# EnriqueOO97/MultiModalVC

Measured on NVIDIA B200. Metric: AV-HuBERT-L encoder 6s-clips/sec, higher is better.
Workload: dtype bf16

## Files before the change

### include/avh_b200.h

```cpp
#ifndef AVH_B200_H_
#define AVH_B200_H_

#include <stdint.h>

#ifdef __cplusplus
extern "C" {
#endif

#define AVH_ABI_VERSION 1
#if defined(__GNUC__)
#define AVH_API __attribute__((visibility("default")))
#else
#define AVH_API
#endif

enum { AVH_F32 = 0, AVH_F16 = 1, AVH_BF16 = 2, AVH_U8 = 3  };
enum {
  AVH_COMPUTE_BF16 = 0,
  AVH_COMPUTE_FP32 = 1
};
enum { AVH_FUSE_CONCAT = 0, AVH_FUSE_ADD = 1 };

typedef struct avh_config {
  int32_t encoder_layers;
// ... 81 lines not shown
                                const int32_t* len_queries, int B, int Lq, int Lk, void* out, int out_dtype, void* stream);

AVH_API int avh_forward_ragged(avh_handle* h, const void* video, int video_dtype, const void* audio, int audio_dtype,
                               const int64_t* audio_strides, const int32_t* lengths, int B, int T, int output_layer,
                               void* out, int out_dtype, void* stream);

AVH_API int avh_set_video_preprocess(avh_handle* h, int src_h, int src_w, double mean, double std);

AVH_API int avh_video_preprocess(const uint8_t* frames, int64_t n_frames, int src_h, int src_w, int crop, double mean,
                         double std, void* out, int out_dtype, void* stream);

AVH_API int avh_forward_host(avh_handle* h, const void* video, int video_dtype, const void* audio, int audio_dtype,
                     const uint8_t* padding_mask, int B, int T, int output_layer, void* out, int out_dtype,
                     void* stream);

AVH_API int avh_forward_host_async(avh_handle* h, const void* video, int video_dtype, const void* audio, int audio_dtype,
                           const uint8_t* padding_mask, int B, int T, int output_layer, void* out, int out_dtype,
                           void* stream);

AVH_API int avh_read_stage(avh_handle* h, const char* name, float* dst, int64_t capacity_elems, void* stream);

AVH_API int avh_fbank(const int16_t* wav, const int64_t* offsets, const int32_t* video_len, int n_clips, int T,
              int normalize, float* out, uint8_t* padding_mask, void* stream);

AVH_API int avh_add_noise(const int16_t* wav, const int64_t* offsets, int n_clips, const float* noise, int64_t noise_len,
                  float snr_db, int16_t* out, double* scratch, void* stream);

AVH_API int avh_attention_bf16(const void* qkv, const uint8_t* padding_mask, const int32_t* cu_rows, int64_t rows, int B,
                               int T, int D, int H, int impl, void* out, void* stream);

AVH_API int avh_gemm_bf16(const void* A, const void* B, int64_t M, int N, int K, const float* bias, int gelu,
                  const void* R, int r_fp32, void* C, int c_fp32, int block_n, int pair, int occ, void* stream);

AVH_API int avh_gemm_set_trace(void* dev_buf);

AVH_API int avh_set_profiling(avh_handle* h, int on);
AVH_API int avh_profile_json(avh_handle* h, char* buf, int64_t cap);

AVH_API int64_t avh_launch_count(void);
AVH_API void avh_reset_launch_count(void);
AVH_API int64_t avh_graph_launch_count(void);

#ifdef __cplusplus
}
#endif
#endif
```

### multimodalvc_b200/_lib.py

```python
import ctypes
import os

_HERE = os.path.dirname(os.path.abspath(__file__))
LIB_PATH = os.path.join(_HERE, "libavh_b200.so")

AVH_F32, AVH_F16, AVH_BF16, AVH_U8 = 0, 1, 2, 3
AVH_COMPUTE_BF16, AVH_COMPUTE_FP32 = 0, 1
AVH_FUSE_CONCAT, AVH_FUSE_ADD = 0, 1

EXPORTS = [
    "avh_abi_version", "avh_last_error", "avh_create", "avh_destroy", "avh_load_tensor", "avh_finalize_weights",
    "avh_forward", "avh_forward_host", "avh_forward_host_async", "avh_read_stage", "avh_fbank", "avh_add_noise", "avh_gemm_bf16",
    "avh_launch_count", "avh_reset_launch_count", "avh_set_profiling", "avh_profile_json",
    "avh_gemm_set_trace", "avh_set_video_preprocess", "avh_video_preprocess", "avh_drop_host_weights",
    "avh_release_stream", "avh_attention_bf16", "avh_forward_ragged", "avh_encoder_forward", "avh_forward_train", "avh_bn_stats_count", "avh_read_bn_stats", "avh_dropout", "avh_interp_linear", "avh_graph_launch_count",
    "avh_mask_substitute", "avh_compute_logits", "avh_sum_squares", "avh_qformer_forward",
    "avh_encoder_grad_count", "avh_encoder_train_forward", "avh_encoder_backward",
    "avh_encoder_backward_buckets", "avh_grad_bucket_count", "avh_grad_bucket_range", "avh_grad_bucket_wait",
    "avh_refresh_weights_device",
    "avh_tail_grad_count", "avh_tail_train_forward", "avh_full_grad_count", "avh_full_train_forward",
]


class AvhConfig(ctypes.Structure):
    _fields_ = [
        ("encoder_layers", ctypes.c_int32),
        ("encoder_embed_dim", ctypes.c_int32),
        ("encoder_ffn_embed_dim", ctypes.c_int32),
        ("encoder_attention_heads", ctypes.c_int32),
        ("audio_feat_dim", ctypes.c_int32),
        ("modality_fuse", ctypes.c_int32),
        ("layer_norm_first", ctypes.c_int32),
        ("conv_pos", ctypes.c_int32),
        ("conv_pos_groups", ctypes.c_int32),
        ("compute_mode", ctypes.c_int32),
        ("frontend_chunk_frames", ctypes.c_int32),
        ("capture_stages", ctypes.c_int32),
        ("reserved", ctypes.c_int32 * 4),
    ]


class AvhTrainArgs(ctypes.Structure):
    _fields_ = [
        ("dropout_input", ctypes.c_float),
        ("dropout", ctypes.c_float),
# ... 30 lines not shown
    lib.avh_forward_ragged.argtypes = [vp, vp, i32, vp, i32, ctypes.POINTER(i64), ctypes.POINTER(ctypes.c_int32), i32, i32, i32, vp,
                                       i32, vp]
    lib.avh_forward_train.argtypes = [vp, vp, i32, vp, i32, ctypes.POINTER(i64), vp, i32, i32, i32, ctypes.POINTER(AvhTrainArgs),
                                      vp, i32, vp]
    lib.avh_interp_linear.argtypes = [vp, i32, i32, i32, i32, vp, vp, i32, vp, vp, vp]
    lib.avh_encoder_grad_count.argtypes = [vp, ctypes.POINTER(i64)]
    lib.avh_tail_grad_count.argtypes = [vp, ctypes.POINTER(i64)]
    lib.avh_full_grad_count.argtypes = [vp, i32, i32, ctypes.POINTER(i64)]
    lib.avh_full_train_forward.argtypes = [vp, vp, i32, vp, i32, ctypes.POINTER(i64), vp, i32, i32, ctypes.c_float, ctypes.c_float,
                                           vp, i32, vp]
    lib.avh_tail_train_forward.argtypes = [vp, vp, i32, vp, i32, i32, vp, i32, vp]
    lib.avh_encoder_train_forward.argtypes = [vp, vp, i32, vp, i32, i32, vp, i32, vp]
    lib.avh_encoder_backward.argtypes = [vp, vp, i32, vp, i32, vp, i64, vp]
    lib.avh_encoder_backward_buckets.argtypes = [vp, vp, i32, vp, i32, vp, i32, i64, vp]
    lib.avh_grad_bucket_count.argtypes = [vp, ctypes.POINTER(ctypes.c_int32)]
    lib.avh_grad_bucket_range.argtypes = [vp, i32, ctypes.POINTER(i64), ctypes.POINTER(i64)]
    lib.avh_grad_bucket_wait.argtypes = [vp, i32, vp]
    lib.avh_refresh_weights_device.argtypes = [vp, ctypes.POINTER(ctypes.c_char_p), ctypes.POINTER(vp), ctypes.POINTER(ctypes.c_int32),
                                               ctypes.POINTER(i64), i32, vp]
    lib.avh_qformer_forward.argtypes = [vp, vp, i32, vp, ctypes.POINTER(ctypes.c_int32), i32, i32, i32, vp, i32, vp]
    lib.avh_mask_substitute.argtypes = [vp, i32, i32, ctypes.POINTER(i64), i32, i32, i32, vp, vp, i32, vp, vp, i32, vp]
    lib.avh_compute_logits.argtypes = [vp, i32, i64, vp, i32, i64, vp, i64, i32, i32, i32, ctypes.c_float, vp, i64, vp]
    lib.avh_sum_squares.argtypes = [vp, i32, i64, vp, vp]
    lib.avh_dropout.argtypes = [vp, i32, i64, ctypes.c_float, ctypes.c_uint64, ctypes.c_uint32, vp]
    lib.avh_bn_stats_count.argtypes = [vp, ctypes.POINTER(i64)]
    lib.avh_read_bn_stats.argtypes = [vp, vp, i64, vp]
    lib.avh_encoder_forward.argtypes = [vp, vp, i32, vp, i32, i32, i32, vp, i32, vp]
    lib.avh_forward_host.argtypes = [vp, vp, i32, vp, i32, vp, i32, i32, i32, vp, i32, vp]
    lib.avh_forward_host_async.argtypes = [vp, vp, i32, vp, i32, vp, i32, i32, i32, vp, i32, vp]
    lib.avh_read_stage.argtypes = [vp, ctypes.c_char_p, vp, i64, vp]
    lib.avh_fbank.argtypes = [vp, vp, vp, i32, i32, i32, vp, vp, vp]
    lib.avh_add_noise.argtypes = [vp, vp, i32, vp, i64, ctypes.c_float, vp, vp, vp]
    lib.avh_gemm_bf16.argtypes = [vp, vp, i64, i32, i32, vp, i32, vp, i32, vp, i32, i32, i32, i32, vp]
    lib.avh_attention_bf16.argtypes = [vp, vp, vp, i64, i32, i32, i32, i32, i32, vp, vp]
    lib.avh_gemm_set_trace.argtypes = [vp]
    lib.avh_set_video_preprocess.argtypes = [vp, i32, i32, ctypes.c_double, ctypes.c_double]
    lib.avh_video_preprocess.argtypes = [vp, i64, i32, i32, i32, ctypes.c_double, ctypes.c_double, vp, i32, vp]
    lib.avh_set_profiling.argtypes = [vp, i32]
    lib.avh_profile_json.argtypes = [vp, ctypes.c_char_p, i64]
    lib.avh_launch_count.restype = i64
    lib.avh_reset_launch_count.restype = None
    lib.avh_graph_launch_count.restype = i64
    for name in EXPORTS:
        fn = getattr(lib, name)
        if fn.restype is ctypes.c_int and name not in ("avh_abi_version",):
            fn.restype = i32
    if lib.avh_abi_version() != 1:
        raise RuntimeError("libavh_b200.so ABI version mismatch; rebuild with `python -m multimodalvc_b200.build --force`")
    _lib = lib
    return lib


def check(status):
    if status != 0:
        msg = load().avh_last_error()
        raise RuntimeError("libavh_b200: " + (msg.decode() if msg else "unknown error"))


def launch_count():
    return int(load().avh_launch_count())


def reset_launch_count():
    load().avh_reset_launch_count()
```

### multimodalvc_b200/csrc/api.cu

```cuda
#include "avh_b200.h"
#include "common.cuh"
#include "gemm.h"
#include "kernels.h"

#include <array>
#include <atomic>
#include <cmath>
#include <cstdlib>
#include <cstring>
#include <functional>
#include <map>
#include <tuple>
#include <memory>
#include <mutex>
#include <string>
#include <vector>

#include <cuda_fp16.h>

namespace avh {

static thread_local std::string g_err;
void set_last_error(const std::string& msg) { g_err = msg; }
static std::atomic<long long> g_launches{0};
// ... 144 lines not shown
  bool has_video = false, has_audio = false, has_mask = false;
  bool train = false;
  float p_in = 0.f, p_enc = 0.f, p_act = 0.f, bn_momentum = 0.1f;
  unsigned long long seed = 0;
  std::vector<unsigned char> layer_skip;
  bool enc_only = false;
  bool enc_train = false;
  int tail = 0;
  size_t fwd_steps = 0;
  float* grads = nullptr;
  long long grad_floats = 0;
  float* dx_out = nullptr;
  float* dy_in = nullptr;
  float fgm = 1.f;
  bool fwd_done = false;
  int Lk = 0;
  unsigned char* qmask_dev = nullptr;
  unsigned char* kmask_dev = nullptr;
  bool ragged = false;
  long long Nb = 0;
  int* rag = nullptr;
  int rag_ints = 0, rag_items_off = 0, rag_max_items = 0;
  static constexpr int RAG_SLOTS = 4;
  int* rag_host[RAG_SLOTS] = {nullptr, nullptr, nullptr, nullptr};
  cudaEvent_t rag_done[RAG_SLOTS] = {nullptr, nullptr, nullptr, nullptr};
  struct GradBucket { long long begin, end; cudaEvent_t ev; };
  std::vector<GradBucket> buckets;
  int rag_next = 0;
  int* pos_row_map = nullptr;

  Arena arena;
  std::vector<Step> steps;
  std::vector<GemmPlan*> gemms;
  std::vector<ConvWinPlan*> convwins;
  std::vector<ConvFramePlan*> convframes;
  StemFusedPlan stemf;
  AttnTcPlan att;
  std::map<std::string, std::pair<const void*, std::pair<int, long long>>> stages;
  CallArgs args;
  struct Segment { size_t begin, end; cudaGraphExec_t exec; int kernels; };
  std::vector<Segment> segments;
  bool segments_ready = false;
  unsigned char* mask_dev = nullptr;
  int direct_runs = 0;
  long long last_use = 0;
  cudaStream_t stream = nullptr;
  void drop_graphs() {
    for (auto& sg : segments)
      if (sg.exec) cudaGraphExecDestroy(sg.exec);
    segments.clear();
    segments_ready = false;
  }
  ~Plan() {
    drop_graphs();
    for (GemmPlan* g : gemms) delete g;
    for (ConvWinPlan* g : convwins) delete g;
    for (ConvFramePlan* g : convframes) delete g;
    for (int i = 0; i < RAG_SLOTS; ++i) {
      if (rag_host[i]) cudaFreeHost(rag_host[i]);
      if (rag_done[i]) cudaEventDestroy(rag_done[i]);
    }
    for (GradBucket& gb : buckets)
      if (gb.ev) cudaEventDestroy(gb.ev);
    arena.release();
  }
};

}
}

using namespace avh;

struct avh_handle {
  avh_config cfg;
  int device = 0;
  int P = 1;
  bool finalized = false;
  std::map<std::string, HostTensor> raw;
  Arena warena;
  ConvUnit stem;
  PackedW stem_wf;
  BlockW blocks[4][2];
  LinearW proj_v, proj_a, post_proj;
  LinearW post_projT;
  LinearW proj_vT;
  bool has_post_proj = false;
  float *fuse_ln_g = nullptr, *fuse_ln_b = nullptr, *enc_ln_g = nullptr, *enc_ln_b = nullptr;
  PackedW pos_w;
// ... 1026 lines not shown
    void* ol = f32 ? nullptr : hbuf.data;
    b.tag = "layer_ln";
    b.push([=](cudaStream_t s) { return launch_layernorm(src, DT_F32, D, g, be, 1e-5f, of, ol, DT_BF16, nullptr, N, D, s); });
    if (f32 && also_f32 != nullptr) {
      float* hd = reinterpret_cast<float*>(hbuf.data);
      b.push([=](cudaStream_t s) {
        return cudaMemcpyAsync(also_f32, hd, (size_t)N * D * 4, cudaMemcpyDeviceToDevice, s) == cudaSuccess ? 0 : 1;
      });
    }
    sync_op(hbuf);
  };
  auto x_to_h = [&]() {
    void* dst = hbuf.op;
    const int planes = P;
    b.tag = "split";
    b.push([=](cudaStream_t s) { return launch_split_rows(x, D, dst, planes, N, D, 0, 0, s); });
  };

  if (!c.layer_norm_first) {
    float* g = h->enc_ln_g; float* be = h->enc_ln_b;
    b.tag = "layer_ln";
    b.push([=](cudaStream_t s) { return launch_layernorm(x, DT_F32, D, g, be, 1e-5f, x, nullptr, DT_BF16, nullptr, N, D, s); });
    if (!train) x_to_h();
  }
  if (train) {
    b.tag = "dropout";
    b.push([=](cudaStream_t s) {
      return pl->p_enc > 0.f ? launch_dropout(x, DT_F32, nullptr, N * D, pl->p_enc, pl->seed, 2u, s) : 0;
    });
    if (!c.layer_norm_first) x_to_h();
  }
  const int n_layers = plan->output_layer > 0 ? std::min(plan->output_layer, c.encoder_layers) : c.encoder_layers;
  const bool att_tc = !f32 && (rg || T > 96) && (size_t)((T + 127) / 128 * 128) * 4 <= 48 * 1024;
  for (int l = 0; l < n_layers; ++l) {
    const LayerW& lw = h->layers[l];
    b.cur_layer = l;
    if (c.layer_norm_first) ln_to_h(x, lw.ln1_g, lw.ln1_b, nullptr);
    {
      Epilogue ep = ep_base(qkv.data, 3 * D);
      ep.col_bias = lw.qkv.bias;
      b.tag = "qkv_proj";
      if (!b.gemm(hbuf.op, N, P * D, lw.qkv.w, N, {Tap{0, 0, 0}}, D / 64, D, ep)) return false;
    }
    {
      const void* q = qkv.data; void* o = ctx.data;
      b.tag = "attention";
      const double att_flops = 4.0 * (double)B * Hh * (double)T * (double)T * 64.0;
      if (att_tc) {
        if (!sizing && l == 0 && attention_tc_plan(q, N, B, T, D, Hh, &plan->att)) return false;
        b.push([=](cudaStream_t s) {
          return attention_tc_launch(pl->att, hm ? pl->mask_dev : nullptr, pl->ragged ? pl->rag + 16 : nullptr, o, s);
        }, att_flops);
      } else {
        b.push([=](cudaStream_t s) {
          return launch_attention(q, hm ? pl->mask_dev : nullptr, o, B, T, D, Hh, f32 ? 1 : 0, s);
        }, att_flops);
      }
      sync_op(ctx);
    }
    auto dropout_add = [&](unsigned site) {
      float* target = c.layer_norm_first ? x : tmp;
      b.tag = "dropout";
      if (!c.layer_norm_first)
        b.push([=](cudaStream_t s) {
          return cudaMemcpyAsync(tmp, x, (size_t)N * D * 4, cudaMemcpyDeviceToDevice, s) == cudaSuccess ? 0 : 1;
        });
      b.push([=](cudaStream_t s) { return launch_dropout(target, DT_F32, dtmp, N * D, pl->p_enc, pl->seed, site, s); });
    };
    {
      Epilogue ep;
      ep.C = c.layer_norm_first ? x : tmp; ep.ldc = D; ep.c_fp32 = 1;
      ep.col_bias = lw.out.bias; ep.R = x; ep.ldr = D; ep.r_fp32 = 1;
      if (train) { ep.C = dtmp; ep.R = nullptr; }
      b.tag = "out_proj";
      if (!b.gemm(ctx.op, N, P * D, lw.out.w, N, {Tap{0, 0, 0}}, D / 64, D, ep)) return false;
      if (train) dropout_add(16u + 4u * (unsigned)l);
    }
    if (c.layer_norm_first) ln_to_h(x, lw.ln2_g, lw.ln2_b, nullptr);
    else {
      float* g = lw.ln1_g; float* be = lw.ln1_b;
      b.tag = "layer_ln";
      b.push([=](cudaStream_t s) { return launch_layernorm(tmp, DT_F32, D, g, be, 1e-5f, x, nullptr, DT_BF16, nullptr, N, D, s); });
      x_to_h();
    }
    {
      Epilogue ep = ep_base(ffn.data, F);
      ep.col_bias = lw.fc1.bias; ep.act = ACT_GELU;
      b.tag = "fc1";
      if (!b.gemm(hbuf.op, N, P * D, lw.fc1.w, N, {Tap{0, 0, 0}}, D / 64, D, ep)) return false;
      if (train) {
        void* fd = ffn.data;
        const unsigned site = 17u + 4u * (unsigned)l;
        b.tag = "dropout";
        b.push([=](cudaStream_t s) {
          return pl->p_act > 0.f ? launch_dropout(fd, act_dt, nullptr, N * F, pl->p_act, pl->seed, site, s) : 0;
        });
      }
      sync_op(ffn);
    }
    {
      Epilogue ep;
      ep.C = c.layer_norm_first ? x : tmp; ep.ldc = D; ep.c_fp32 = 1;
      ep.col_bias = lw.fc2.bias; ep.R = x; ep.ldr = D; ep.r_fp32 = 1;
      if (train) { ep.C = dtmp; ep.R = nullptr; }
      b.tag = "fc2";
      if (!b.gemm(ffn.op, N, P * F, lw.fc2.w, N, {Tap{0, 0, 0}}, F / 64, F, ep)) return false;
      if (train) dropout_add(18u + 4u * (unsigned)l);
    }
    if (!c.layer_norm_first) {
      float* g = lw.ln2_g; float* be = lw.ln2_b;
      b.tag = "layer_ln";
      b.push([=](cudaStream_t s) { return launch_layernorm(tmp, DT_F32, D, g, be, 1e-5f, x, nullptr, DT_BF16, nullptr, N, D, s); });
      if (l + 1 < n_layers) x_to_h();
    }
  }
  b.cur_layer = -1;
  b.tag = "final_ln";
  if (rg) {
    float* y = x;
    if (c.layer_norm_first && plan->output_layer == 0) {
      y = reinterpret_cast<float*>(b.alloc((size_t)N * D * 4));
      float* g = h->enc_ln_g; float* be = h->enc_ln_b;
      b.push([=](cudaStream_t s) { return launch_layernorm(x, DT_F32, D, g, be, 1e-5f, y, nullptr, DT_BF16, nullptr, N, D, s); });
    }
    b.tag = "unpack";
    b.cur_direct = true;
    b.push([=](cudaStream_t s) {
      return launch_unpack_rows(y, pl->rag + 16, pl->args.out, pl->args.out_dt, B, pl->args.pitch, D, s);
    });
  } else
  if (c.layer_norm_first && plan->output_layer == 0) {
    b.cur_direct = true;
    float* g = h->enc_ln_g; float* be = h->enc_ln_b;
    b.push([=](cudaStream_t s) {
      return launch_layernorm(x, DT_F32, D, g, be, 1e-5f, nullptr, pl->args.out, pl->args.out_dt, nullptr, N, D, s);
    });
  } else {
    b.cur_direct = true;
    b.push([=](cudaStream_t s) { return launch_convert(x, DT_F32, pl->args.out, pl->args.out_dt, N * D, s); });
  }
// ... 2020 lines not shown
    std::vector<avh::KStep> t;
    for (int i = 0; i < kb0 * r; ++i) t.push_back(avh::KStep{(i % kb0) * 64, 0, (i % kb0) * 64, 0});
    if (d_ktab == nullptr) AVH_CUDA_OK(cudaMalloc(&d_ktab, avh::GEMM_MAX_KSTEPS * sizeof(avh::KStep)));
    AVH_CUDA_OK(cudaMemcpy(d_ktab, t.data(), t.size() * sizeof(avh::KStep), cudaMemcpyHostToDevice));
    pr.ktable = reinterpret_cast<const avh::KStep*>(d_ktab);
    pr.num_kb = kb0 * r;
  }
  pr.block_n = block_n;
  pr.pair = pair;
  pr.occ = occ;
  {
    static std::map<int, std::pair<float*, int*>> ws;
    int dev = 0;
    AVH_CUDA_OK(cudaGetDevice(&dev));
    const size_t bytes = (size_t)avh::device_sm_count() * 128 * 256 * 4;
    if (ws.find(dev) == ws.end()) {
      float* w = nullptr; int* f = nullptr;
      AVH_CUDA_OK(cudaMalloc(&w, bytes));
      AVH_CUDA_OK(cudaMalloc(&f, 4096));
      AVH_CUDA_OK(cudaMemset(f, 0, 4096));
      ws[dev] = {w, f};
    }
    pr.sk_ws = ws[dev].first; pr.sk_ws_bytes = bytes; pr.sk_flags = ws[dev].second;
  }
  pr.ep.C = C; pr.ep.ldc = N; pr.ep.c_fp32 = c_fp32;
  pr.ep.col_bias = bias;
  pr.ep.act = gelu ? avh::ACT_GELU : avh::ACT_NONE;
  pr.ep.R = R; pr.ep.ldr = N; pr.ep.r_fp32 = r_fp32;
  avh::GemmPlan plan;
  if (avh::gemm_plan(pr, &plan)) return 1;
  return avh::gemm_launch(plan, reinterpret_cast<cudaStream_t>(stream));
}

}
```

### multimodalvc_b200/csrc/gemm.h

```cpp
#pragma once
#include <cuda.h>
#include <cuda_runtime.h>
#include <vector_types.h>
#include <stdint.h>

#include <vector>

namespace avh {

enum { ACT_NONE = 0, ACT_GELU = 1, ACT_PRELU = 2 };
enum { MAP_IDENTITY = 0, MAP_2LEVEL = 1 };

struct Epilogue {
  void* C = nullptr;
  long long ldc = 0;
  int c_fp32 = 0;
  const float* col_scale = nullptr;
  const float* col_bias = nullptr;
  int act = ACT_NONE;
  const float* slope1 = nullptr;
  const void* R = nullptr;
  long long ldr = 0;
  int r_fp32 = 0;
  const float* slope2 = nullptr;
// ... 86 lines not shown
struct ConvFramePlan {
  CUtensorMap tma_a, tma_b, tma_c, tma_a2;
  ConvFrameProblem prob;
  int grid = 0, stages = 0, pair = 1;
  size_t smem = 0;
  std::vector<int> tiles_host;
  const int* tiles_dev = nullptr;
};
int conv_frame_plan(const ConvFrameProblem& prob, ConvFramePlan* plan);
size_t conv_frame_table_bytes(const ConvFrameProblem& prob);
int conv_frame_bind_table(ConvFramePlan* plan, void* dev_table);
int conv_frame_launch(const ConvFramePlan& plan, cudaStream_t stream);
struct StemFusedPlan {
  const void* w = nullptr;
};
int stem_fused_plan(const void* w_packed, StemFusedPlan* plan);
int stem_fused_launch(const StemFusedPlan& plan, const void* video, int in_dt, int T, int b0, int nb, const float* scale,
                      const float* bias, const float* slope, void* pooled_out, cudaStream_t stream);
struct AttnTcPlan {
  CUtensorMap tma_q, tma_kv;
  int B = 0, T = 0, D = 0, H = 0;
  int kv_rows = 0, stages = 0, stage_bytes = 0, mask_floats = 0;
  size_t smem = 0;
};
int attention_tc_plan(const void* qkv, long long rows, int B, int T, int D, int H, AttnTcPlan* plan);
int attention_tc_launch(const AttnTcPlan& plan, const unsigned char* kpm, const int* cu, void* out, cudaStream_t stream);
int stem_fused_ragged_items(const int* lengths, int n_clips, int sms, int4* items, int max_items);
int stem_fused_launch_ragged(const StemFusedPlan& plan, const void* video, int in_dt, int Tpitch, const int4* items,
                             const int* n_items, const int* cu, const float* scale, const float* bias, const float* slope,
                             void* out, cudaStream_t stream);
int encode_2d(CUtensorMap* map, const void* base, long long rows, int cols, long long ld, int box_rows);
int encode_c(CUtensorMap* map, const void* base, long long rows, int cols, long long ld, int fp32);

constexpr int GEMM_MAX_KSTEPS = 768;

int gemm_plan(const GemmProblem& prob, GemmPlan* plan);
int gemm_launch(const GemmPlan& plan, cudaStream_t stream);
int gemm_pick_block_n(long long M, int N);
void gemm_set_trace(unsigned long long* dev_buf);

}
```

### multimodalvc_b200/csrc/gemm_tcgen05.cu

```cuda
#include "common.cuh"
#include "gemm.h"

#include <cstdlib>
#include <mutex>
#include <set>

namespace avh {

namespace {

constexpr int BM = 128;
constexpr int BK = 64;
constexpr int A_STAGE_BYTES = BM * BK * 2;
constexpr int MAX_STAGES = 8;
constexpr int COLVEC_BYTES = 2 * 4 * 256 * 4;
constexpr int BAR_BYTES = (2 * MAX_STAGES + 4) * 8 + 16;

template <int OCC>
struct Occ {
  static constexpr int EPI_WARPS = OCC == 2 ? 4 : 8;
  static constexpr int NUM_THREADS = 128 + 32 * EPI_WARPS;
  static constexpr int TMEM_COLS = 512 / OCC;
  static constexpr int ACC_STRIDE = 256 / OCC;
  static constexpr int EPI_STAGE_BYTES = EPI_WARPS * 4096;
  static constexpr int SMEM_LIMIT = OCC == 2 ? 113 * 1024 : 227 * 1024;
  static constexpr int HSTRIDE = EPI_WARPS / 4;
};

struct KernelParams {
  long long M;
  int N;
  int num_kb;
  int num_m_blk, num_n_blk;
  int block_n;
  int stages;
  int ktab_bytes;
  int a_col_per_nblk;
  const int* a_col_nblk;
// ... 569 lines not shown
          __syncwarp();
        }
        if (half >= nchunks) {
          tc_fence_before();
          __syncwarp();
          if (lane == 0) {
            if (PAIR == 2) mbar_arrive_leader(&tmem_empty[acc]);
            else mbar_arrive(&tmem_empty[acc]);
          }
        }
      }
      if (warp == 4 && lane == 0) {
        if (it == 0) AVH_TRACE(7);
        AVH_TRACE(9);
      }
      if (SK != 0 && sk_last >= sk_first) {
        asm volatile("bar.sync 1, %0;" ::"n"(32 * EPI_WARPS) : "memory");
        if (threadIdx.x == 128)
          for (int v = sk_first; v <= sk_last; ++v) p.sk_flags[v * PAIR + cta_rank] = 0;
      }
    }
    if (lane == 0 && p.c_mode != 0) tma_wait_group0();
  }

  tc_fence_before();
  if (PAIR == 2) cluster_sync_all();
  else __syncthreads();
  tc_fence_after();
  if (threadIdx.x == 0) AVH_TRACE(10);
  if (warp == 2) {
    if (PAIR == 2) tmem_dealloc_pair(tmem_base, TMEM_COLS);
    else tmem_dealloc(tmem_base, TMEM_COLS);
    if (lane == 0) AVH_TRACE(11);
  }
}

typedef CUresult (*EncodeTiledFn)(CUtensorMap*, CUtensorMapDataType, cuuint32_t, void*, const cuuint64_t*,
                                  const cuuint64_t*, const cuuint32_t*, const cuuint32_t*, CUtensorMapInterleave,
                                  CUtensorMapSwizzle, CUtensorMapL2promotion, CUtensorMapFloatOOBfill);

EncodeTiledFn get_encode_fn() {
  static EncodeTiledFn fn = nullptr;
  if (fn == nullptr) {
    void* p = nullptr;
    cudaDriverEntryPointQueryResult q;
    if (cudaGetDriverEntryPoint("cuTensorMapEncodeTiled", &p, cudaEnableDefault, &q) == cudaSuccess &&
        q == cudaDriverEntryPointSuccess)
      fn = reinterpret_cast<EncodeTiledFn>(p);
  }
  return fn;
}

}

int encode_c(CUtensorMap* map, const void* base, long long rows, int cols, long long ld, int fp32) {
  EncodeTiledFn fn = get_encode_fn();
  AVH_CHECK(fn != nullptr, "cuTensorMapEncodeTiled entry point not available");
  const int es = fp32 ? 4 : 2;
  AVH_CHECK((reinterpret_cast<uintptr_t>(base) & 15) == 0 && (ld * es) % 16 == 0, "TMA store alignment");
  cuuint64_t dims[2] = {(cuuint64_t)cols, (cuuint64_t)rows};
  cuuint64_t strides[1] = {(cuuint64_t)ld * es};
  cuuint32_t box[2] = {(cuuint32_t)(128 / es), 32u};
  cuuint32_t estr[2] = {1, 1};
  CUresult r = fn(map, fp32 ? CU_TENSOR_MAP_DATA_TYPE_FLOAT32 : CU_TENSOR_MAP_DATA_TYPE_BFLOAT16, 2,
                  const_cast<void*>(base), dims, strides, box, estr, CU_TENSOR_MAP_INTERLEAVE_NONE,
                  CU_TENSOR_MAP_SWIZZLE_128B, CU_TENSOR_MAP_L2_PROMOTION_NONE, CU_TENSOR_MAP_FLOAT_OOB_FILL_NONE);
// ... 214 lines not shown
    fn = gemm_kernel<1, O, A, R, S, C, F>;
  AVH_SPEC(1, ACT_NONE, 0, 0, 0, 0)
  AVH_SPEC(1, ACT_NONE, 0, 0, 0, 1)
  AVH_SPEC(1, ACT_GELU, 0, 0, 0, 0)
  AVH_SPEC(1, ACT_GELU, 0, 0, 0, 1)
  AVH_SPEC(1, ACT_NONE, 1, 0, 0, 1)
  AVH_SPEC(1, ACT_GELU, 1, 0, 0, 1)
  AVH_SPEC(1, ACT_PRELU, 0, 0, 1, 0)
  AVH_SPEC(1, ACT_PRELU, 0, 0, 1, 1)
  AVH_SPEC(1, ACT_NONE, 1, 1, 1, 0)
  AVH_SPEC(1, ACT_NONE, 1, 1, 1, 1)
  AVH_SPEC(1, ACT_NONE, 0, 0, 1, 0)
  AVH_SPEC(1, ACT_NONE, 0, 0, 1, 1)
  AVH_SPEC(2, ACT_NONE, 0, 0, 0, 0)
  AVH_SPEC(2, ACT_NONE, 0, 0, 0, 1)
  AVH_SPEC(2, ACT_GELU, 0, 0, 0, 0)
  AVH_SPEC(2, ACT_NONE, 1, 0, 0, 1)
  AVH_SPEC(2, ACT_GELU, 1, 0, 0, 1)
  AVH_SPEC(2, ACT_PRELU, 0, 0, 1, 0)
  AVH_SPEC(2, ACT_NONE, 1, 1, 1, 0)
  AVH_SPEC(2, ACT_NONE, 0, 0, 1, 0)
#undef AVH_SPEC
  if (fn == nullptr) {
    if (pair == 2) fn = gemm_kernel<2, 1, -1, -1, -1, -1, -1>;
    else if (occ == 2) fn = gemm_kernel<1, 2, -1, -1, -1, -1, -1>;
    else fn = gemm_kernel<1, 1, -1, -1, -1, -1, -1>;
  }
  if (ensure_dyn_smem(reinterpret_cast<const void*>(fn), occ == 2 ? Occ<2>::SMEM_LIMIT : Occ<1>::SMEM_LIMIT)) return 1;
  AVH_CUDA_OK(cudaLaunchKernelEx(&cfg, fn, plan.tma_a, plan.tma_b, plan.tma_c, kp));
  count_launch(1);
  return 0;
}

}
```

Before: 4232.

## Fuse FFN fc1 and fc2 into one persistent kernel with row-level dependencies

Replaces the two separate fc1 (GELU) and fc2 (bias plus residual) GEMM launches in inference with a single persistent tcgen05 kernel. Tiles come from an atomic work queue and are interleaved with a planned lag, so fc2 tiles for an M row-block start once all of that block's fc1 tiles are published through per-row release/acquire counters. This removes the inter-kernel drain and tail between the two GEMMs and lets the two phases overlap. The cost is spin-waiting, a global atomic scheduler, a self-resetting sync buffer, and a heuristic tile-size and lag model.

```diff
diff --git a/include/avh_b200.h b/include/avh_b200.h
--- a/include/avh_b200.h
+++ b/include/avh_b200.h
@@ -137,6 +137,9 @@
 AVH_API int avh_gemm_bf16(const void* A, const void* B, int64_t M, int N, int K, const float* bias, int gelu,
                   const void* R, int r_fp32, void* C, int c_fp32, int block_n, int pair, int occ, void* stream);
 
+AVH_API int avh_ffn_bf16(const void* h, const void* W1, const float* b1, const void* W2, const float* b2, void* ffn_out,
+                         float* x, float* out, int64_t M, int D, int F, int block_n1, int block_n2, void* stream);
+
 AVH_API int avh_gemm_set_trace(void* dev_buf);
 
 AVH_API int avh_set_profiling(avh_handle* h, int on);
diff --git a/multimodalvc_b200/_lib.py b/multimodalvc_b200/_lib.py
--- a/multimodalvc_b200/_lib.py
+++ b/multimodalvc_b200/_lib.py
@@ -10,7 +10,7 @@
 
 EXPORTS = [
     "avh_abi_version", "avh_last_error", "avh_create", "avh_destroy", "avh_load_tensor", "avh_finalize_weights",
-    "avh_forward", "avh_forward_host", "avh_forward_host_async", "avh_read_stage", "avh_fbank", "avh_add_noise", "avh_gemm_bf16",
+    "avh_forward", "avh_forward_host", "avh_forward_host_async", "avh_read_stage", "avh_fbank", "avh_add_noise", "avh_gemm_bf16", "avh_ffn_bf16",
     "avh_launch_count", "avh_reset_launch_count", "avh_set_profiling", "avh_profile_json",
     "avh_gemm_set_trace", "avh_set_video_preprocess", "avh_video_preprocess", "avh_drop_host_weights",
     "avh_release_stream", "avh_attention_bf16", "avh_forward_ragged", "avh_encoder_forward", "avh_forward_train", "avh_bn_stats_count", "avh_read_bn_stats", "avh_dropout", "avh_interp_linear", "avh_graph_launch_count",
@@ -107,6 +107,7 @@
     lib.avh_fbank.argtypes = [vp, vp, vp, i32, i32, i32, vp, vp, vp]
     lib.avh_add_noise.argtypes = [vp, vp, i32, vp, i64, ctypes.c_float, vp, vp, vp]
     lib.avh_gemm_bf16.argtypes = [vp, vp, i64, i32, i32, vp, i32, vp, i32, vp, i32, i32, i32, i32, vp]
+    lib.avh_ffn_bf16.argtypes = [vp, vp, vp, vp, vp, vp, vp, vp, i64, i32, i32, i32, i32, vp]
     lib.avh_attention_bf16.argtypes = [vp, vp, vp, i64, i32, i32, i32, i32, i32, vp, vp]
     lib.avh_gemm_set_trace.argtypes = [vp]
     lib.avh_set_video_preprocess.argtypes = [vp, i32, i32, ctypes.c_double, ctypes.c_double]
diff --git a/multimodalvc_b200/csrc/api.cu b/multimodalvc_b200/csrc/api.cu
--- a/multimodalvc_b200/csrc/api.cu
+++ b/multimodalvc_b200/csrc/api.cu
@@ -200,6 +200,7 @@
   Arena arena;
   std::vector<Step> steps;
   std::vector<GemmPlan*> gemms;
+  std::vector<FfnPlan*> ffns;
   std::vector<ConvWinPlan*> convwins;
   std::vector<ConvFramePlan*> convframes;
   StemFusedPlan stemf;
@@ -222,6 +223,7 @@
   ~Plan() {
     drop_graphs();
     for (GemmPlan* g : gemms) delete g;
+    for (FfnPlan* g : ffns) delete g;
     for (ConvWinPlan* g : convwins) delete g;
     for (ConvFramePlan* g : convframes) delete g;
     for (int i = 0; i < RAG_SLOTS; ++i) {
@@ -1314,6 +1316,8 @@
   }
   const int n_layers = plan->output_layer > 0 ? std::min(plan->output_layer, c.encoder_layers) : c.encoder_layers;
   const bool att_tc = !f32 && (rg || T > 96) && (size_t)((T + 127) / 128 * 128) * 4 <= 48 * 1024;
+  const bool ffn_fused = !train && !f32 && D % 64 == 0 && F % 64 == 0 && !h->layers.empty() &&
+                         h->layers[0].fc1.w.kpad == D && h->layers[0].fc2.w.kpad == F;
   for (int l = 0; l < n_layers; ++l) {
     const LayerW& lw = h->layers[l];
     b.cur_layer = l;
@@ -1365,29 +1369,45 @@
       b.push([=](cudaStream_t s) { return launch_layernorm(tmp, DT_F32, D, g, be, 1e-5f, x, nullptr, DT_BF16, nullptr, N, D, s); });
       x_to_h();
     }
-    {
-      Epilogue ep = ep_base(ffn.data, F);
-      ep.col_bias = lw.fc1.bias; ep.act = ACT_GELU;
-      b.tag = "fc1";
-      if (!b.gemm(hbuf.op, N, P * D, lw.fc1.w, N, {Tap{0, 0, 0}}, D / 64, D, ep)) return false;
-      if (train) {
-        void* fd = ffn.data;
-        const unsigned site = 17u + 4u * (unsigned)l;
-        b.tag = "dropout";
-        b.push([=](cudaStream_t s) {
-          return pl->p_act > 0.f ? launch_dropout(fd, act_dt, nullptr, N * F, pl->p_act, pl->seed, site, s) : 0;
-        });
+    if (ffn_fused) {
+      int* sync = reinterpret_cast<int*>(b.alloc((size_t)ffn_sync_ints(N) * 4));
+      b.tag = "ffn";
+      if (!sizing) {
+        FfnProblem fp;
+        fp.h = hbuf.op; fp.w1 = lw.fc1.w.w; fp.b1 = lw.fc1.bias; fp.w2 = lw.fc2.w.w; fp.b2 = lw.fc2.bias;
+        fp.ffn = ffn.data; fp.x = x; fp.out = c.layer_norm_first ? nullptr : tmp;
+        fp.M = N; fp.D = D; fp.F = F;
+        fp.sync = sync;
+        FfnPlan* fpl = new FfnPlan();
+        plan->ffns.push_back(fpl);
+        if (ffn_plan(fp, fpl)) return false;
+        b.push([fpl](cudaStream_t s) { return ffn_launch(*fpl, s); }, 2.0 * 2.0 * (double)N * (double)D * (double)F);
       }
-      sync_op(ffn);
-    }
-    {
-      Epilogue ep;
-      ep.C = c.layer_norm_first ? x : tmp; ep.ldc = D; ep.c_fp32 = 1;
-      ep.col_bias = lw.fc2.bias; ep.R = x; ep.ldr = D; ep.r_fp32 = 1;
-      if (train) { ep.C = dtmp; ep.R = nullptr; }
-      b.tag = "fc2";
-      if (!b.gemm(ffn.op, N, P * F, lw.fc2.w, N, {Tap{0, 0, 0}}, F / 64, F, ep)) return false;
-      if (train) dropout_add(18u + 4u * (unsigned)l);
+    } else {
+      {
+        Epilogue ep = ep_base(ffn.data, F);
+        ep.col_bias = lw.fc1.bias; ep.act = ACT_GELU;
+        b.tag = "fc1";
+        if (!b.gemm(hbuf.op, N, P * D, lw.fc1.w, N, {Tap{0, 0, 0}}, D / 64, D, ep)) return false;
+        if (train) {
+          void* fd = ffn.data;
+          const unsigned site = 17u + 4u * (unsigned)l;
+          b.tag = "dropout";
+          b.push([=](cudaStream_t s) {
+            return pl->p_act > 0.f ? launch_dropout(fd, act_dt, nullptr, N * F, pl->p_act, pl->seed, site, s) : 0;
+          });
+        }
+        sync_op(ffn);
+      }
+      {
+        Epilogue ep;
+        ep.C = c.layer_norm_first ? x : tmp; ep.ldc = D; ep.c_fp32 = 1;
+        ep.col_bias = lw.fc2.bias; ep.R = x; ep.ldr = D; ep.r_fp32 = 1;
+        if (train) { ep.C = dtmp; ep.R = nullptr; }
+        b.tag = "fc2";
+        if (!b.gemm(ffn.op, N, P * F, lw.fc2.w, N, {Tap{0, 0, 0}}, F / 64, F, ep)) return false;
+        if (train) dropout_add(18u + 4u * (unsigned)l);
+      }
     }
     if (!c.layer_norm_first) {
       float* g = lw.ln2_g; float* be = lw.ln2_b;
@@ -3474,4 +3494,37 @@
   return avh::gemm_launch(plan, reinterpret_cast<cudaStream_t>(stream));
 }
 
-}
+int avh_ffn_bf16(const void* h, const void* W1, const float* b1, const void* W2, const float* b2, void* ffn_out,
+                 float* x, float* out, int64_t M, int D, int F, int block_n1, int block_n2, void* stream) {
+  avh::FfnProblem pr;
+  pr.h = h; pr.w1 = W1; pr.b1 = b1; pr.w2 = W2; pr.b2 = b2;
+  pr.ffn = ffn_out; pr.x = x; pr.out = out;
+  pr.M = M; pr.D = D; pr.F = F;
+  pr.block_n1 = block_n1; pr.block_n2 = block_n2;
+  cudaStream_t s = reinterpret_cast<cudaStream_t>(stream);
+  {
+    static std::mutex mu;
+    static std::map<std::pair<int, cudaStream_t>, std::pair<int*, int>> counters;
+    std::lock_guard<std::mutex> lock(mu);
+    int dev = 0;
+    AVH_CUDA_OK(cudaGetDevice(&dev));
+    const int need = avh::ffn_sync_ints(M);
+    auto& e = counters[{dev, s}];
+    if (e.second < need) {
+      if (e.first != nullptr) {
+        AVH_CUDA_OK(cudaStreamSynchronize(s));
+        AVH_CUDA_OK(cudaFree(e.first));
+        e = {nullptr, 0};
+      }
+      AVH_CUDA_OK(cudaMalloc(&e.first, (size_t)need * 4));
+      AVH_CUDA_OK(cudaMemset(e.first, 0, (size_t)need * 4));
+      e.second = need;
+    }
+    pr.sync = e.first;
+  }
+  avh::FfnPlan plan;
+  if (avh::ffn_plan(pr, &plan)) return 1;
+  return avh::ffn_launch(plan, s);
+}
+
+}
diff --git a/multimodalvc_b200/csrc/gemm.h b/multimodalvc_b200/csrc/gemm.h
--- a/multimodalvc_b200/csrc/gemm.h
+++ b/multimodalvc_b200/csrc/gemm.h
@@ -142,6 +142,30 @@
 int encode_2d(CUtensorMap* map, const void* base, long long rows, int cols, long long ld, int box_rows);
 int encode_c(CUtensorMap* map, const void* base, long long rows, int cols, long long ld, int fp32);
 
+struct FfnProblem {
+  const void* h = nullptr;
+  const void* w1 = nullptr;
+  const float* b1 = nullptr;
+  const void* w2 = nullptr;
+  const float* b2 = nullptr;
+  void* ffn = nullptr;
+  float* x = nullptr;
+  float* out = nullptr;
+  long long M = 0;
+  int D = 0, F = 0;
+  int block_n1 = 0, block_n2 = 0;
+  int* sync = nullptr;
+};
+struct FfnPlan {
+  CUtensorMap tma_a0, tma_b0, tma_c0, tma_a1, tma_b1, tma_c1;
+  FfnProblem prob;
+  int grid = 0, stages = 0, b_stride = 0, lag = 0, total = 0;
+  size_t smem = 0;
+};
+int ffn_sync_ints(long long M);
+int ffn_plan(const FfnProblem& prob, FfnPlan* plan);
+int ffn_launch(const FfnPlan& plan, cudaStream_t stream);
+
 constexpr int GEMM_MAX_KSTEPS = 768;
 
 int gemm_plan(const GemmProblem& prob, GemmPlan* plan);
diff --git a/multimodalvc_b200/csrc/gemm_tcgen05.cu b/multimodalvc_b200/csrc/gemm_tcgen05.cu
--- a/multimodalvc_b200/csrc/gemm_tcgen05.cu
+++ b/multimodalvc_b200/csrc/gemm_tcgen05.cu
@@ -1,9 +1,13 @@
 #include "common.cuh"
 #include "gemm.h"
 
+#include <algorithm>
+#include <array>
 #include <cstdlib>
+#include <map>
 #include <mutex>
 #include <set>
+#include <vector>
 
 namespace avh {
 
@@ -639,6 +643,328 @@
     if (PAIR == 2) tmem_dealloc_pair(tmem_base, TMEM_COLS);
     else tmem_dealloc(tmem_base, TMEM_COLS);
     if (lane == 0) AVH_TRACE(11);
+  }
+}
+
+constexpr int FFN_RING = 8;
+
+struct FfnParams {
+  long long M;
+  int num_m_blk;
+  int n0, n1;
+  int N0, N1;
+  int kb0, kb1;
+  int bn0, bn1;
+  int stages;
+  int b_stride;
+  int lag;
+  int total;
+  int c_mode1;
+  const float* bias0;
+  const float* bias1;
+  const float* R;
+  int* sync;
+};
+
+struct FfnTile { int phase, m_blk, n_blk; };
+
+__device__ __forceinline__ FfnTile ffn_tile(const FfnParams& p, int idx) {
+  const int n0 = p.n0, n1 = p.n1, L = p.lag;
+  if (idx < L * n0) return FfnTile{0, idx / n0, idx % n0};
+  idx -= L * n0;
+  const int gs = n0 + n1, G = p.num_m_blk - L;
+  if (idx < G * gs) {
+    const int g = idx / gs, o = idx - g * gs;
+    return o < n0 ? FfnTile{0, g + L, o} : FfnTile{1, g, o - n0};
+  }
+  idx -= G * gs;
+  return FfnTile{1, G + idx / n1, idx % n1};
+}
+
+template <int PH>
+__device__ __forceinline__ void ffn_epilogue(const CUtensorMap* tma_c, const FfnParams& p, int BN, int n_blk, int row0,
+                                             uint32_t taddr, const float* cv, uint8_t* stg, int half, int lane,
+                                             uint64_t* tmem_empty) {
+  constexpr int BOX = PH ? 32 : 64;
+  constexpr int HSTRIDE = Occ<1>::HSTRIDE;
+  const int N = PH ? p.N1 : p.N0;
+  const bool has_res = PH == 1 && p.c_mode1 == 1;
+  const long long r = (long long)row0 + lane;
+  const bool live = r < p.M;
+  const int nboxes = BN / BOX;
+#pragma unroll 1
+  for (int bx = half; bx < nboxes; bx += HSTRIDE) {
+    const int cbase = bx * BOX;
+    uint32_t packed[32];
+#pragma unroll
+    for (int sub = 0; sub < BOX / 32; ++sub) {
+      const int c0 = cbase + sub * 32;
+      const int col0 = n_blk * BN + c0;
+      uint32_t rawv[32];
+      tmem_ld_32x32(taddr + c0, rawv);
+      uint4 rres[8];
+      if (has_res && live && col0 < N) {
+        const uint4* rp = reinterpret_cast<const uint4*>(p.R + r * N + col0);
+#pragma unroll
+        for (int j = 0; j < 8; ++j) rres[j] = __ldg(rp + j);
+      }
+      tmem_ld_wait();
+      float v[32];
+#pragma unroll
+      for (int j = 0; j < 32; ++j) v[j] = __uint_as_float(rawv[j]);
+      if (col0 < N) {
+#pragma unroll
+        for (int j = 0; j < 8; ++j) {
+          const float4 bi = *reinterpret_cast<const float4*>(cv + c0 + 4 * j);
+          v[4 * j] += bi.x; v[4 * j + 1] += bi.y; v[4 * j + 2] += bi.z; v[4 * j + 3] += bi.w;
+        }
+        if (PH == 0) {
+#pragma unroll
+          for (int j = 0; j < 32; ++j) v[j] = gelu_erf_fast(v[j]);
+        }
+        if (has_res && live) {
+#pragma unroll
+          for (int j = 0; j < 8; ++j) {
+            v[4 * j] += __uint_as_float(rres[j].x); v[4 * j + 1] += __uint_as_float(rres[j].y);
+            v[4 * j + 2] += __uint_as_float(rres[j].z); v[4 * j + 3] += __uint_as_float(rres[j].w);
+          }
+        }
+      }
+      if (PH == 1) {
+#pragma unroll
+        for (int j = 0; j < 32; ++j) packed[j] = __float_as_uint(v[j]);
+      } else {
+#pragma unroll
+        for (int j = 0; j < 16; ++j) packed[sub * 16 + j] = pack_bf16(v[2 * j], v[2 * j + 1]);
+      }
+    }
+    if (bx + HSTRIDE >= nboxes) {
+      tc_fence_before();
+      __syncwarp();
+      if (lane == 0) mbar_arrive(tmem_empty);
+    }
+    if (lane == 0) tma_wait_group_read0();
+    __syncwarp();
+#pragma unroll
+    for (int j = 0; j < 8; ++j)
+      *reinterpret_cast<uint4*>(stg + lane * 128 + ((j ^ (lane & 7)) << 4)) =
+          make_uint4(packed[4 * j], packed[4 * j + 1], packed[4 * j + 2], packed[4 * j + 3]);
+    fence_proxy_async_smem();
+    __syncwarp();
+    if (lane == 0) {
+      if (row0 < p.M) {
+        if (PH == 1 && p.c_mode1 == 2) tma_reduce_add_2d(tma_c, stg, n_blk * BN + cbase, row0);
+        else tma_store_2d(tma_c, stg, n_blk * BN + cbase, row0);
+      }
+      tma_commit_group();
+    }
+  }
+  if (half >= nboxes) {
+    tc_fence_before();
+    __syncwarp();
+    if (lane == 0) mbar_arrive(tmem_empty);
+  }
+}
+
+__global__ void __launch_bounds__(Occ<1>::NUM_THREADS, 1)
+ffn_kernel(const __grid_constant__ CUtensorMap tma_a0, const __grid_constant__ CUtensorMap tma_b0,
+           const __grid_constant__ CUtensorMap tma_c0, const __grid_constant__ CUtensorMap tma_a1,
+           const __grid_constant__ CUtensorMap tma_b1, const __grid_constant__ CUtensorMap tma_c1, const FfnParams p) {
+  constexpr int EPI_WARPS = Occ<1>::EPI_WARPS;
+  constexpr int ACC_STRIDE = Occ<1>::ACC_STRIDE;
+  constexpr int TMEM_COLS = Occ<1>::TMEM_COLS;
+  extern __shared__ uint8_t smem_raw[];
+  const uint32_t raw = smem_u32(smem_raw);
+  uint8_t* smem = smem_raw + (((raw + 1023u) & ~1023u) - raw);
+  const int STAGES = p.stages;
+  uint8_t* smem_a = smem;
+  uint8_t* smem_b = smem + STAGES * A_STAGE_BYTES;
+  uint8_t* epi_stage = smem_b + STAGES * p.b_stride;
+  float* colvec = reinterpret_cast<float*>(epi_stage + Occ<1>::EPI_STAGE_BYTES);
+  uint64_t* full_bar = reinterpret_cast<uint64_t*>(reinterpret_cast<uint8_t*>(colvec) + COLVEC_BYTES);
+  uint64_t* empty_bar = full_bar + MAX_STAGES;
+  uint64_t* tmem_full = empty_bar + MAX_STAGES;
+  uint64_t* tmem_empty = tmem_full + 2;
+  uint64_t* ring_full = tmem_empty + 2;
+  uint64_t* ring_empty = ring_full + FFN_RING;
+  int* ring_id = reinterpret_cast<int*>(ring_empty + FFN_RING);
+  uint32_t* tmem_slot = reinterpret_cast<uint32_t*>(ring_id + FFN_RING);
+
+  const int warp = threadIdx.x >> 5;
+  const int lane = threadIdx.x & 31;
+  pdl_launch_dependents();
+  if (warp == 0 && lane == 0) {
+    tma_prefetch_desc(&tma_a0); tma_prefetch_desc(&tma_b0); tma_prefetch_desc(&tma_c0);
+    tma_prefetch_desc(&tma_a1); tma_prefetch_desc(&tma_b1); tma_prefetch_desc(&tma_c1);
+  }
+  if (warp == 1 && lane == 0) {
+    for (int s = 0; s < STAGES; ++s) {
+      mbar_init(&full_bar[s], 1);
+      mbar_init(&empty_bar[s], 1);
+    }
+    for (int s = 0; s < 2; ++s) {
+      mbar_init(&tmem_full[s], 1);
+      mbar_init(&tmem_empty[s], EPI_WARPS);
+    }
+    for (int s = 0; s < FFN_RING; ++s) {
+      mbar_init(&ring_full[s], 1);
+      mbar_init(&ring_empty[s], 1 + EPI_WARPS);
+    }
+    mbar_fence_init();
+  }
+  if (warp == 2) tmem_alloc(tmem_slot, TMEM_COLS);
+  if (warp == 0 && (int)blockIdx.x < p.total) {
+    const FfnTile t0 = ffn_tile(p, blockIdx.x);
+    if (t0.phase == 0 && elect_one()) {
+      const int pre = p.kb0 < STAGES ? p.kb0 : STAGES;
+      for (int kb = 0; kb < pre; ++kb)
+        asm volatile("cp.async.bulk.prefetch.tensor.2d.L2.global.tile [%0, {%1, %2}];"
+                     ::"l"(reinterpret_cast<uint64_t>(&tma_b0)), "r"(kb * BK), "r"(t0.n_blk * p.bn0) : "memory");
+    }
+    __syncwarp();
+  }
+  tc_fence_before();
+  __syncthreads();
+  tc_fence_after();
+  const uint32_t tmem_base = *tmem_slot;
+  pdl_wait();
+
+  if (warp == 0) {
+    int stage = 0;
+    uint32_t phase = 0;
+    for (int it = 0;; ++it) {
+      int idx = 0;
+      if (lane == 0) idx = atomicAdd(p.sync, 1);
+      idx = __shfl_sync(0xffffffffu, idx, 0);
+      const int slot = it % FFN_RING;
+      mbar_wait(&ring_empty[slot], ((it / FFN_RING) & 1) ^ 1);
+      if (lane == 0) {
+        ring_id[slot] = idx < p.total ? idx : -1;
+        mbar_arrive(&ring_full[slot]);
+      }
+      __syncwarp();
+      if (idx >= p.total) break;
+      const FfnTile t = ffn_tile(p, idx);
+      const CUtensorMap* ta = t.phase ? &tma_a1 : &tma_a0;
+      const CUtensorMap* tb = t.phase ? &tma_b1 : &tma_b0;
+      const int BN = t.phase ? p.bn1 : p.bn0;
+      const int nkb = t.phase ? p.kb1 : p.kb0;
+      if (t.phase == 1) {
+        if (lane == 0) {
+          const int* cnt = p.sync + 2 + t.m_blk;
+          int v, ns = 32;
+          while (true) {
+            asm volatile("ld.acquire.gpu.global.b32 %0, [%1];" : "=r"(v) : "l"(cnt) : "memory");
+            if (v >= p.n0) break;
+            __nanosleep(ns);
+            if (ns < 512) ns *= 2;
+          }
+          asm volatile("fence.proxy.async.global;" ::: "memory");
+        }
+        __syncwarp();
+      }
+      const uint32_t stage_tx = (uint32_t)(A_STAGE_BYTES + BN * BK * 2);
+      const int m0 = t.m_blk * BM, n0 = t.n_blk * BN;
+      for (int kb = 0; kb < nkb; ++kb) {
+        mbar_wait(&empty_bar[stage], phase ^ 1);
+        if (elect_one()) {
+          mbar_expect_tx(&full_bar[stage], stage_tx);
+          tma_load_2d(smem_a + stage * A_STAGE_BYTES, ta, &full_bar[stage], kb * BK, m0);
+          tma_load_2d(smem_b + stage * p.b_stride, tb, &full_bar[stage], kb * BK, n0);
+        }
+        __syncwarp();
+        if (++stage == STAGES) { stage = 0; phase ^= 1; }
+      }
+    }
+  } else if (warp == 1) {
+    int stage = 0;
+    uint32_t phase = 0;
+    for (int it = 0;; ++it) {
+      const int slot = it % FFN_RING;
+      mbar_wait(&ring_full[slot], (it / FFN_RING) & 1);
+      const int idx = ring_id[slot];
+      __syncwarp();
+      if (lane == 0) mbar_arrive(&ring_empty[slot]);
+      if (idx < 0) break;
+      const FfnTile t = ffn_tile(p, idx);
+      const int BN = t.phase ? p.bn1 : p.bn0;
+      const int nkb = t.phase ? p.kb1 : p.kb0;
+      const uint32_t idesc = umma_idesc_bf16(BM, BN);
+      const int acc = it & 1;
+      mbar_wait(&tmem_empty[acc], ((it >> 1) & 1) ^ 1);
+      tc_fence_after();
+      const uint32_t tmem_d = tmem_base + acc * ACC_STRIDE;
+      for (int kb = 0; kb < nkb; ++kb) {
+        mbar_wait(&full_bar[stage], phase);
+        tc_fence_after();
+        const uint64_t adesc = umma_desc_sw128(smem_u32(smem_a + stage * A_STAGE_BYTES));
+        const uint64_t bdesc = umma_desc_sw128(smem_u32(smem_b + stage * p.b_stride));
+        if (elect_one()) {
+#pragma unroll
+          for (int k = 0; k < BK / 16; ++k) umma_bf16(tmem_d, adesc + 2 * k, bdesc + 2 * k, idesc, (kb > 0) || (k != 0));
+          umma_commit(&empty_bar[stage]);
+        }
+        __syncwarp();
+        if (++stage == STAGES) { stage = 0; phase ^= 1; }
+      }
+      if (elect_one()) umma_commit(&tmem_full[acc]);
+      __syncwarp();
+    }
+  } else if (warp >= 4) {
+    const int q = warp & 3;
+    const int half = (warp - 4) >> 2;
+    uint8_t* stg = epi_stage + (warp - 4) * 4096;
+    for (int it = 0;; ++it) {
+      const int slot = it % FFN_RING;
+      mbar_wait(&ring_full[slot], (it / FFN_RING) & 1);
+      const int idx = ring_id[slot];
+      __syncwarp();
+      if (lane == 0) mbar_arrive(&ring_empty[slot]);
+      if (idx < 0) break;
+      const FfnTile t = ffn_tile(p, idx);
+      const int BN = t.phase ? p.bn1 : p.bn0;
+      const int N = t.phase ? p.N1 : p.N0;
+      const float* bias = t.phase ? p.bias1 : p.bias0;
+      const int acc = it & 1;
+      const int row0 = t.m_blk * BM + q * 32;
+      float* cv = colvec + acc * 1024;
+      for (int c = threadIdx.x - 128; c < 256; c += 32 * EPI_WARPS) {
+        const int gc = t.n_blk * BN + c;
+        cv[c] = (c < BN && gc < N) ? __ldg(bias + gc) : 0.f;
+      }
+      asm volatile("bar.sync 1, %0;" ::"n"(32 * EPI_WARPS) : "memory");
+      mbar_wait(&tmem_full[acc], (it >> 1) & 1);
+      tc_fence_after();
+      const uint32_t taddr = tmem_base + ((uint32_t)(q * 32) << 16) + acc * ACC_STRIDE;
+      if (t.phase == 0) {
+        ffn_epilogue<0>(&tma_c0, p, BN, t.n_blk, row0, taddr, cv, stg, half, lane, &tmem_empty[acc]);
+        if (lane == 0) {
+          tma_wait_group0();
+          asm volatile("fence.proxy.async.global;" ::: "memory");
+        }
+        __syncwarp();
+        asm volatile("bar.sync 1, %0;" ::"n"(32 * EPI_WARPS) : "memory");
+        if (threadIdx.x == 128)
+          asm volatile("red.release.gpu.global.add.s32 [%0], 1;" ::"l"(p.sync + 2 + t.m_blk) : "memory");
+      } else {
+        ffn_epilogue<1>(&tma_c1, p, BN, t.n_blk, row0, taddr, cv, stg, half, lane, &tmem_empty[acc]);
+      }
+    }
+    if (lane == 0) tma_wait_group0();
+  }
+
+  tc_fence_before();
+  __syncthreads();
+  tc_fence_after();
+  if (warp == 2) tmem_dealloc(tmem_base, TMEM_COLS);
+  if (threadIdx.x == 0) {
+    __threadfence();
+    if (atomicAdd(p.sync + 1, 1) == (int)gridDim.x - 1) {
+      __threadfence();
+      for (int r = 0; r < p.num_m_blk; ++r) atomicExch(p.sync + 2 + r, 0);
+      atomicExch(p.sync, 0);
+      atomicExch(p.sync + 1, 0);
+    }
   }
 }
 
@@ -919,4 +1245,136 @@
   return 0;
 }
 
-}
+namespace {
+
+constexpr int FFN_BAR_BYTES = 512;
+
+int ffn_pick_bn(long long M, int N, int num_kb, int out_f32, int sms) {
+  const int step = out_f32 ? 32 : 64;
+  double best = 1e30;
+  int bn = step;
+  for (int c = step; c <= 256 && c <= ((N + step - 1) / step) * step; c += step) {
+    const double t = model_cycles(M, N, num_kb, c, 1, 1, sms, 0, out_f32);
+    if (t < best) { best = t; bn = c; }
+  }
+  return bn;
+}
+
+int ffn_pick_lag(int mb, int n0, int n1, double t0, double t1, int sms) {
+  int best_lag = mb;
+  double best = 1e30;
+  std::vector<double> free_at(sms), row_done(mb);
+  for (int L = 1; L <= mb; ++L) {
+    std::fill(free_at.begin(), free_at.end(), 0.0);
+    std::fill(row_done.begin(), row_done.end(), 0.0);
+    double end = 0.0;
+    auto run = [&](int phase, int r) {
+      auto it = std::min_element(free_at.begin(), free_at.end());
+      const double fin = phase == 0 ? *it + t0 : std::max(*it, row_done[r]) + t1;
+      if (phase == 0) row_done[r] = std::max(row_done[r], fin);
+      *it = fin;
+      end = std::max(end, fin);
+    };
+    for (int r = 0; r < L; ++r)
+      for (int n = 0; n < n0; ++n) run(0, r);
+    for (int g = 0; g < mb - L; ++g) {
+      for (int n = 0; n < n0; ++n) run(0, g + L);
+      for (int n = 0; n < n1; ++n) run(1, g);
+    }
+    for (int r = mb - L; r < mb; ++r)
+      for (int n = 0; n < n1; ++n) run(1, r);
+    if (end < best - 1.0) { best = end; best_lag = L; }
+  }
+  return best_lag;
+}
+
+double ffn_kblock_cycles(int bn) {
+  double k = 415.0;
+  if (2.0 * bn > k) k = 2.0 * bn;
+  const double ingress = (double)(A_STAGE_BYTES + bn * BK * 2) / 66.0;
+  return ingress > k ? ingress : k;
+}
+
+}
+
+int ffn_sync_ints(long long M) { return 2 + (int)((M + BM - 1) / BM); }
+
+int ffn_plan(const FfnProblem& pr, FfnPlan* plan) {
+  AVH_CHECK(pr.h && pr.w1 && pr.w2 && pr.b1 && pr.b2 && pr.ffn && pr.x && pr.sync, "null pointer");
+  AVH_CHECK(pr.D % 64 == 0 && pr.F % 64 == 0, "D and F must be multiples of 64");
+  AVH_CHECK(pr.M >= 1 && pr.M < (1ll << 31) - 2 * BM, "M out of range");
+  AVH_CHECK(pr.block_n1 >= 0 && pr.block_n1 <= 256 && pr.block_n1 % 64 == 0, "block_n1 must be a multiple of 64, <= 256");
+  AVH_CHECK(pr.block_n2 >= 0 && pr.block_n2 <= 256 && pr.block_n2 % 32 == 0, "block_n2 must be a multiple of 32, <= 256");
+  plan->prob = pr;
+  const int sms = device_sm_count();
+  const int bn0 = pr.block_n1 ? pr.block_n1 : ffn_pick_bn(pr.M, pr.F, pr.D / 64, 0, sms);
+  const int bn1 = pr.block_n2 ? pr.block_n2 : ffn_pick_bn(pr.M, pr.D, pr.F / 64, 1, sms);
+  plan->prob.block_n1 = bn0;
+  plan->prob.block_n2 = bn1;
+  if (encode_2d(&plan->tma_a0, pr.h, pr.M, pr.D, pr.D, BM)) return 1;
+  if (encode_2d(&plan->tma_b0, pr.w1, pr.F, pr.D, pr.D, bn0)) return 1;
+  if (encode_c(&plan->tma_c0, pr.ffn, pr.M, pr.F, pr.F, 0)) return 1;
+  if (encode_2d(&plan->tma_a1, pr.ffn, pr.M, pr.F, pr.F, BM)) return 1;
+  if (encode_2d(&plan->tma_b1, pr.w2, pr.D, pr.F, pr.F, bn1)) return 1;
+  if (encode_c(&plan->tma_c1, pr.out ? pr.out : pr.x, pr.M, pr.D, pr.D, 1)) return 1;
+  const int mb = (int)((pr.M + BM - 1) / BM);
+  const int n0 = (pr.F + bn0 - 1) / bn0, n1 = (pr.D + bn1 - 1) / bn1;
+  plan->total = mb * (n0 + n1);
+  plan->grid = std::min(plan->total, sms);
+  {
+    static std::mutex mu;
+    static std::map<std::array<int, 8>, int> lags;
+    const std::array<int, 8> key{mb, n0, n1, bn0, bn1, pr.D, pr.F, plan->grid};
+    std::lock_guard<std::mutex> lock(mu);
+    auto it = lags.find(key);
+    if (it == lags.end())
+      it = lags.emplace(key, ffn_pick_lag(mb, n0, n1, (pr.D / 64) * ffn_kblock_cycles(bn0) + 300.0,
+                                          (pr.F / 64) * ffn_kblock_cycles(bn1) + 300.0, plan->grid)).first;
+    plan->lag = it->second;
+  }
+  plan->b_stride = std::max(bn0, bn1) * BK * 2;
+  int stages = (Occ<1>::SMEM_LIMIT - 1024 - Occ<1>::EPI_STAGE_BYTES - COLVEC_BYTES - FFN_BAR_BYTES) /
+               (A_STAGE_BYTES + plan->b_stride);
+  if (stages > MAX_STAGES) stages = MAX_STAGES;
+  AVH_CHECK(stages >= 2, "tile too large for shared memory");
+  plan->stages = stages;
+  plan->smem = 1024 + (size_t)stages * (A_STAGE_BYTES + plan->b_stride) + Occ<1>::EPI_STAGE_BYTES + COLVEC_BYTES +
+               FFN_BAR_BYTES;
+  return 0;
+}
+
+int ffn_launch(const FfnPlan& plan, cudaStream_t stream) {
+  const FfnProblem& pr = plan.prob;
+  FfnParams kp;
+  kp.M = pr.M;
+  kp.num_m_blk = (int)((pr.M + BM - 1) / BM);
+  kp.bn0 = pr.block_n1; kp.bn1 = pr.block_n2;
+  kp.N0 = pr.F; kp.N1 = pr.D;
+  kp.n0 = (pr.F + kp.bn0 - 1) / kp.bn0; kp.n1 = (pr.D + kp.bn1 - 1) / kp.bn1;
+  kp.kb0 = pr.D / 64; kp.kb1 = pr.F / 64;
+  kp.stages = plan.stages;
+  kp.b_stride = plan.b_stride;
+  kp.lag = plan.lag;
+  kp.total = plan.total;
+  kp.c_mode1 = pr.out ? 1 : 2;
+  kp.bias0 = pr.b1; kp.bias1 = pr.b2;
+  kp.R = pr.x;
+  kp.sync = pr.sync;
+  cudaLaunchConfig_t cfg = {};
+  cfg.gridDim = dim3((unsigned)plan.grid);
+  cfg.blockDim = dim3(Occ<1>::NUM_THREADS);
+  cfg.dynamicSmemBytes = plan.smem;
+  cfg.stream = stream;
+  cudaLaunchAttribute attr[1];
+  attr[0].id = cudaLaunchAttributeProgrammaticStreamSerialization;
+  attr[0].val.programmaticStreamSerializationAllowed = 1;
+  cfg.attrs = attr;
+  cfg.numAttrs = pdl_enabled() ? 1 : 0;
+  if (ensure_dyn_smem(reinterpret_cast<const void*>(ffn_kernel), Occ<1>::SMEM_LIMIT)) return 1;
+  AVH_CUDA_OK(cudaLaunchKernelEx(&cfg, ffn_kernel, plan.tma_a0, plan.tma_b0, plan.tma_c0, plan.tma_a1, plan.tma_b1,
+                                 plan.tma_c1, kp));
+  count_launch(1);
+  return 0;
+}
+
+}
```

New measurement: 4247 (median of 6 runs). About the same (+0.4%).
